# zju3dv/pvnet

Hardware: NVIDIA H100
Metric: images/sec (480x640, K=9) backbone+vote (higher is better)
Workload: dtype tf32 (fp32 storage, fp32 accumulate; vote fp32/fp64)

## Files before the change

### pvnet_b200/csrc/vote.cu

```cuda
#include "common.cuh"

#include <cfloat>
#include <cmath>

namespace {

using pvnet::Carver;

constexpr int CH_PX = 2048;
constexpr int CH_THREADS = 256;
constexpr int VT_THREADS = 256;
constexpr int VT_WARPS = VT_THREADS / 32;
constexpr int VT_TILE = 512;
constexpr int VT_MAX_B = 1024;
constexpr int RF_CHUNKS = 8;
constexpr int RF_THREADS = 256;

struct Strides {
    long long s[5];
};

__device__ __forceinline__ bool exact_inlier(float nx, float ny, float cx, float cy, float hx, float hy,
                                             float thresh)
{
    const float dx = __fsub_rn(hx, cx);
    const float dy = __fsub_rn(hy, cy);
    const float norm1 = __fsqrt_rn(__fmaf_rn(nx, nx, __fmul_rn(ny, ny)));
    const float norm2 = __fsqrt_rn(__fmaf_rn(dx, dx, __fmul_rn(dy, dy)));
    if (fmin((double)norm1, (double)norm2) < 1e-6) return false;
    const float num = __fmaf_rn(dx, nx, __fmul_rn(dy, ny));
    const float den = __fmul_rn(norm1, norm2);
    const float ang = __fdiv_rn(num, den);
    return ang > thresh;
}

__device__ __forceinline__ float2 exact_hypothesis(float d0x, float d0y, float cx0, float cy0, float d1x,
                                                   float d1y, float cx1, float cy1)
{
    const float p = __fmul_rn(d0y, d1x);
    const float q = __fmul_rn(d0x, d1y);
    const float det_y = __fsub_rn(p, q);
    if ((double)fabsf(det_y) < 1e-6) return make_float2(0.f, 0.f);
    const float det_x = __fsub_rn(q, p);
    if ((double)fabsf(det_x) < 1e-6) return make_float2(0.f, 0.f);
    const float s1 = __fmaf_rn(d1y, cx1, -__fmul_rn(d1x, cy1));
    const float s0 = __fmaf_rn(d0y, cx0, -__fmul_rn(d0x, cy0));
    const float y = __fdiv_rn(__fmaf_rn(d1y, s0, -__fmul_rn(d0y, s1)), det_y);
    const float x = __fdiv_rn(__fmaf_rn(-d1x, s0, __fmul_rn(d0x, s1)), det_x);
    return make_float2(x, y);
}

__device__ __forceinline__ int warp_sum(int v)
{
#pragma unroll
    for (int o = 16; o > 0; o >>= 1) v += __shfl_xor_sync(0xffffffffu, v, o);
    return v;
}

__device__ __forceinline__ void block_sum3(int &a, int &b, int &c, int *scratch )
{
    const int lane = threadIdx.x & 31, warp = threadIdx.x >> 5, nw = (blockDim.x + 31) >> 5;
    a = warp_sum(a);
    b = warp_sum(b);
    c = warp_sum(c);
    __syncthreads();
    if (lane == 0) {
        scratch[warp] = a;
        scratch[32 + warp] = b;
        scratch[64 + warp] = c;
    }
    __syncthreads();
    int ta = 0, tb = 0, tc = 0;
    for (int i = 0; i < nw; ++i) {
        ta += scratch[i];
        tb += scratch[32 + i];
        tc += scratch[64 + i];
    }
    a = ta;
    b = tb;
    c = tc;
}

template <typename T>
__device__ __forceinline__ bool is_foreground(T v, int mode)
{
    if (mode == PVNET_MASK_EQUALS_ONE) return v == (T)1;
    return (unsigned char)v != 0;
}

__device__ __forceinline__ float subsample_p(int fg, int max_num)
{
    return __fmul_rn(__frcp_rn((float)fg), (float)max_num);
}

__device__ __forceinline__ uint4 philox4x32_10(uint4 c, uint2 k)
{
#pragma unroll
    for (int r = 0; r < 10; ++r) {
        const unsigned hi0 = __umulhi(0xD2511F53u, c.x), lo0 = 0xD2511F53u * c.x;
        const unsigned hi1 = __umulhi(0xCD9E8D57u, c.z), lo1 = 0xCD9E8D57u * c.z;
        c = make_uint4(hi1 ^ c.y ^ k.x, lo1, hi0 ^ c.w ^ k.y, lo0);
        k.x += 0x9E3779B9u;
        k.y += 0xBB67AE85u;
    }
    return c;
}
enum { RNG_SELECTION = 0, RNG_IDXS_V3 = 1, RNG_IDXS_COV = 2, RNG_IDXS_CENTER = 3 };
__device__ __forceinline__ uint4 rng_draw(const unsigned long long *__restrict__ rng_state, unsigned item,
                                          unsigned image, unsigned stream)
{
    const unsigned long long seed = rng_state[0], off = rng_state[1];
    return philox4x32_10(make_uint4(item, image | (stream << 28), (unsigned)off, (unsigned)(off >> 32)),
                         make_uint2((unsigned)seed, (unsigned)(seed >> 32)));
}
__device__ __forceinline__ float selection_value(const float *__restrict__ sel_field,
                                                 const unsigned long long *__restrict__ rng_state, int b, int npx, int i)
{
    if (sel_field) return sel_field[(size_t)b * npx + i];
    return (float)(rng_draw(rng_state, (unsigned)i, (unsigned)b, RNG_SELECTION).x & 0xffffffu) * 5.9604644775390625e-8f;
}
__global__ void k_rng_bump(unsigned long long *rng_state) { rng_state[1] += 1ull; }

template <typename T>
__global__ void __launch_bounds__(CH_THREADS) k_chunk_count(const T *__restrict__ mask, int mode, int npx,
                                                             int nchunk, int *__restrict__ chunk_fg)
{
    __shared__ int scratch[96];
    const int c = blockIdx.x, b = blockIdx.y;
    const T *m = mask + (size_t)b * npx;
    const int base = c * CH_PX + threadIdx.x * 8;
    int cnt = 0;
#pragma unroll
    for (int j = 0; j < 8; ++j) {
        const int i = base + j;
        if (i < npx) cnt += is_foreground(m[i], mode) ? 1 : 0;
    }
    int z0 = 0, z1 = 0;
    block_sum3(cnt, z0, z1, scratch);
    if (threadIdx.x == 0) chunk_fg[b * nchunk + c] = cnt;
}

template <typename T>
__global__ void __launch_bounds__(CH_THREADS)
    k_chunk_kept(const T *__restrict__ mask, int mode, const float *__restrict__ selection,
                 const unsigned long long *__restrict__ rng_state, int npx, int nchunk, int min_num, int max_num,
                 const int *__restrict__ chunk_fg, int *__restrict__ chunk_kept, int *__restrict__ status)
{
    __shared__ int scratch[96];
    const int c = blockIdx.x, b = blockIdx.y;
    int tot = 0, z0 = 0, z1 = 0;
    for (int i = threadIdx.x; i < nchunk; i += blockDim.x) tot += chunk_fg[b * nchunk + i];
    block_sum3(tot, z0, z1, scratch);
    const bool skip = tot < min_num;
    const bool have_sel = selection != nullptr || rng_state != nullptr;
    const bool sub = tot > max_num && !skip;
    if (!sub || !have_sel) {
        if (threadIdx.x == 0) {
            chunk_kept[b * nchunk + c] = skip ? 0 : chunk_fg[b * nchunk + c];
            if (c == 0) status[b] = (skip ? 1 : 0) | ((sub && !have_sel) ? 4 : 0);
        }
        return;
    }
    const float p = subsample_p(tot, max_num);
    const T *m = mask + (size_t)b * npx;
    const int base = c * CH_PX + threadIdx.x * 8;
    int cnt = 0;
#pragma unroll
    for (int j = 0; j < 8; ++j) {
        const int i = base + j;
        if (i < npx) cnt += (is_foreground(m[i], mode) && selection_value(selection, rng_state, b, npx, i) < p) ? 1 : 0;
    }
    block_sum3(cnt, z0, z1, scratch);
    if (threadIdx.x == 0) {
        chunk_kept[b * nchunk + c] = cnt;
        if (c == 0) status[b] = 2;
    }
}

template <typename T>
__global__ void __launch_bounds__(CH_THREADS)
    k_compact_write(const T *__restrict__ mask, int mode, const float *__restrict__ selection,
                    const unsigned long long *__restrict__ rng_state, int npx, int width, int nchunk, int min_num,
                    int max_num, const int *__restrict__ chunk_fg, const int *__restrict__ chunk_kept_or_null,
                    unsigned *__restrict__ pix, int *__restrict__ tn_out, int *__restrict__ fg_out)
{
    __shared__ int scratch[96];
    __shared__ int warp_off[CH_THREADS / 32];
    const int c = blockIdx.x, b = blockIdx.y;
    const int *chunk_kept = chunk_kept_or_null ? chunk_kept_or_null : chunk_fg;
    int tot_fg = 0, prefix = 0, tot_kept = 0;
    for (int i = threadIdx.x; i < nchunk; i += blockDim.x) {
        const int k = chunk_kept[b * nchunk + i];
        tot_fg += chunk_fg[b * nchunk + i];
        tot_kept += k;
        if (i < c) prefix += k;
    }
    block_sum3(tot_fg, prefix, tot_kept, scratch);
    if (!chunk_kept_or_null && tot_fg < min_num) tot_kept = 0;
    if (c == 0 && threadIdx.x == 0) {
        tn_out[b] = tot_kept;
        fg_out[b] = tot_fg;
    }
    if (tot_kept == 0 || chunk_kept[b * nchunk + c] == 0) return;
    const bool sub = (tot_fg > max_num) && chunk_kept_or_null && (selection != nullptr || rng_state != nullptr);
    const float p = sub ? subsample_p(tot_fg, max_num) : 0.f;
    const T *m = mask + (size_t)b * npx;
    const int base = c * CH_PX + threadIdx.x * 8;
    unsigned flags = 0;
#pragma unroll
    for (int j = 0; j < 8; ++j) {
        const int i = base + j;
        if (i < npx) {
            bool keep = is_foreground(m[i], mode);
            if (sub && keep) keep = selection_value(selection, rng_state, b, npx, i) < p;
            flags |= (keep ? 1u : 0u) << j;
        }
    }
    const int mine = __popc(flags);
    const int lane = threadIdx.x & 31, warp = threadIdx.x >> 5;
    int inc = mine;
#pragma unroll
    for (int o = 1; o < 32; o <<= 1) {
        const int v = __shfl_up_sync(0xffffffffu, inc, o);
        if (lane >= o) inc += v;
    }
    if (lane == 31) warp_off[warp] = inc;
    __syncthreads();
    int woff = 0;
    for (int i = 0; i < warp; ++i) woff += warp_off[i];
    int r = prefix + woff + inc - mine;
    unsigned *out = pix + (size_t)b * npx;
#pragma unroll
    for (int j = 0; j < 8; ++j) {
        if (flags & (1u << j)) {
            const int i = base + j;
            const int y = i / width, x = i - y * width;
            out[r++] = ((unsigned)y << 16) | (unsigned)x;
        }
    }
}

__global__ void k_sum_chunks(const int *__restrict__ chunk_fg, int nchunk, int *__restrict__ fg_out)
{
    __shared__ int scratch[96];
    const int b = blockIdx.x;
    int tot = 0, z0 = 0, z1 = 0;
    for (int i = threadIdx.x; i < nchunk; i += blockDim.x) tot += chunk_fg[b * nchunk + i];
    block_sum3(tot, z0, z1, scratch);
    if (threadIdx.x == 0) fg_out[b] = tot;
}

__global__ void __launch_bounds__(256)
    k_gather(const float *__restrict__ vertex, Strides st, const unsigned *__restrict__ pix,
             const int *__restrict__ tn_arr, int npx, int cap, int vn, float2 *__restrict__ direct)
{
    const int g = blockIdx.x, b = blockIdx.y, tid = threadIdx.x;
    const int tn = tn_arr[b];
    const int t0 = g * VT_TILE;
    if (t0 >= tn) return;
    const int len = min(VT_TILE, tn - t0);
    const bool vec2 = st.s[4] == 1 && ((st.s[0] | st.s[1] | st.s[2] | st.s[3]) & 1) == 0 &&
                      (reinterpret_cast<uintptr_t>(vertex) & 7) == 0;
    for (int i = tid; i < len; i += 256) {
        const unsigned p = pix[(size_t)b * npx + t0 + i];
        const int x = p & 0xffff, y = p >> 16;
        const long long base = (long long)b * st.s[0] + (long long)y * st.s[1] + (long long)x * st.s[2];
        float2 *o = direct + (size_t)b * vn * cap + t0 + i;
        for (int k = 0; k < vn; ++k) {
            const long long off = base + (long long)k * st.s[3];
            float2 v;
            if (vec2) v = __ldg(reinterpret_cast<const float2 *>(vertex + off));
            else v = make_float2(__ldg(vertex + off), __ldg(vertex + off + st.s[4]));
            o[(size_t)k * cap] = v;
        }
    }
}

template <bool SEG>
__device__ __forceinline__ int seg_image(int b, int seg_div) { return SEG ? b / seg_div : b; }
template <bool SEG>
__device__ __forceinline__ int seg_start(const int *seg_off, int b) { return SEG ? seg_off[b] : 0; }

template <bool SEG>
__global__ void __launch_bounds__(256)
    k_gen_hyp(const float2 *__restrict__ direct, const int *__restrict__ idxs,
              const unsigned long long *__restrict__ rng_state, int rng_stream, const unsigned *__restrict__ pix,
              const int *__restrict__ tn_arr, int npx, int cap, int vn, int hn, int HT, int h_off,
              float2 *__restrict__ hyp, const int *__restrict__ seg_off, int seg_div)
{
    const int i = blockIdx.x * blockDim.x + threadIdx.x;
    const int b = blockIdx.y;
    if (i >= hn * vn) return;
    const int hi = i / vn, vi = i - hi * vn;
    const int tn = tn_arr[b];
    float2 out = make_float2(0.f, 0.f);
    if (tn > 0) {
        unsigned t0, t1;
        if (idxs) {
            const size_t ib = (((size_t)b * hn + hi) * vn + vi) * 2;
            t0 = (unsigned)idxs[ib] % (unsigned)tn;
            t1 = (unsigned)idxs[ib + 1] % (unsigned)tn;
        } else {
            const uint4 r = rng_draw(rng_state, (unsigned)i, (unsigned)b, (unsigned)rng_stream);
            t0 = r.x % (unsigned)tn;
            t1 = r.y % (unsigned)tn;
        }
        const int fb = seg_image<SEG>(b, seg_div);
        const int so = seg_start<SEG>(seg_off, b);
        const unsigned *pb = pix + (size_t)fb * npx + so;
        const float2 *db = direct + ((size_t)fb * vn + vi) * cap + so;
        const unsigned p0 = pb[t0], p1 = pb[t1];
        const float2 d0 = db[t0], d1 = db[t1];
        out = exact_hypothesis(d0.x, d0.y, (float)(p0 & 0xffff), (float)(p0 >> 16), d1.x, d1.y, (float)(p1 & 0xffff),
                               (float)(p1 >> 16));
    }
    hyp[((size_t)b * vn + vi) * HT + h_off + hi] = out;
}

typedef unsigned long long f32x2;
__device__ __forceinline__ f32x2 pk2(float a, float b)
{
    f32x2 r;
    asm("mov.b64 %0, {%1, %2};" : "=l"(r) : "f"(a), "f"(b));
    return r;
}
__device__ __forceinline__ void upk2(f32x2 v, float &a, float &b)
{
    asm("mov.b64 {%0, %1}, %2;" : "=f"(a), "=f"(b) : "l"(v));
}
__device__ __forceinline__ f32x2 fma2(f32x2 a, f32x2 b, f32x2 c)
{
    float a0, a1, b0, b1, c0, c1;
    upk2(a, a0, a1);
    upk2(b, b0, b1);
    upk2(c, c0, c1);
    return pk2(__fmaf_rn(a0, b0, c0), __fmaf_rn(a1, b1, c1));
}
__device__ __forceinline__ void lds_2x64(uint32_t addr, f32x2 &a, f32x2 &b)
{
    asm volatile("ld.shared.v2.b64 {%0, %1}, [%2];" : "=l"(a), "=l"(b) : "r"(addr));
}
__device__ __forceinline__ uint32_t ptx_smem_u32(const void *p) { return (uint32_t)__cvta_generic_to_shared(p); }
constexpr int VT_SUB = 64;

__device__ __forceinline__ float min3_nan_abs(float a, float b, float c)
{
    float r;
    asm("{\n\t.reg .f32 t;\n\tmin.NaN.f32 t, %1, %2;\n\tmin.NaN.f32 %0, t, %3;\n\t}" : "=f"(r) : "f"(a), "f"(fabsf(b)), "f"(fabsf(c)));
    return r;
}

template <int HPL, bool SEGMENTED>
__global__ void __launch_bounds__(VT_THREADS, HPL > 4 ? 2 : 3)
    k_vote3(const unsigned *__restrict__ pix, const float2 *__restrict__ direct, const int *__restrict__ tn_arr, int npx,
            int cap, int nb, int vn, int hn, int HT, int h0, const float2 *__restrict__ hyp, int *__restrict__ counts,
            unsigned *__restrict__ ticket, float thresh, float sn, float cs, float beta, float b0, int items_per_warp,
            const int *__restrict__ seg_off, int seg_div)
{
    constexpr int G = 4;
    static_assert(G % 2 == 0 && VT_SUB % G == 0, "pixels are swept in pairs");
    __shared__ float4 rec_all[VT_WARPS * 3 * VT_SUB];
    __shared__ int seg_prefix[VT_MAX_B + 1];
    __shared__ int s_seg;

    const int tid = threadIdx.x, lane = tid & 31, warp = tid >> 5;
    const int HC = 32 * HPL;
    const int hcn = (hn + HC - 1) / HC;
    if (tid == 0) {
        long long px = 0;
        for (int i = 0; i < nb; ++i) px += tn_arr[i];
        const long long want = (long long)gridDim.x * VT_WARPS * items_per_warp;
        int seg = 4096;
        while (seg > 4 * VT_SUB && (px / seg + nb) * vn * hcn < want) seg >>= 1;
        int acc = 0;
        for (int i = 0; i < nb; ++i) {
            seg_prefix[i] = acc;
            acc += (tn_arr[i] + seg - 1) / seg;
        }
        seg_prefix[nb] = acc;
        s_seg = seg;
    }
    __syncthreads();
    const int SEG = s_seg;
    const long long n_items = (long long)seg_prefix[nb] * vn * hcn;
    const float qnan = __int_as_float(0x7fc00000);
    const float finf = __int_as_float(0x7f800000);
    float4 *rec = rec_all + warp * (3 * VT_SUB);
    const uint32_t rec_u = ptx_smem_u32(rec);

    for (;;) {
        unsigned item_u = 0;
        if (lane == 0) item_u = atomicAdd(ticket, 1u);
        const long long it = (long long)__shfl_sync(0xffffffffu, item_u, 0);
        if (it >= n_items) break;
        const int hc = (int)(it % hcn);
        const long long r = it / hcn;
        const int k = (int)(r % vn);
        const int g = (int)(r / vn);
        int lo = 0, hi = nb;
        while (hi - lo > 1) {
            const int mid = (lo + hi) >> 1;
            if (seg_prefix[mid] <= g) lo = mid; else hi = mid;
        }
        const int b = lo;
        const int tn = tn_arr[b];
        const int t0 = (g - seg_prefix[b]) * SEG;
        const int len = min(SEG, tn - t0);
        const int fb = seg_image<SEGMENTED>(b, seg_div);
        const int so = seg_start<SEGMENTED>(seg_off, b) + t0;
        const unsigned *pix_t = pix + (size_t)fb * npx + so;
        const float2 *dir_t = direct + ((size_t)fb * vn + k) * cap + so;

        const int hbase = hc * HC;
        const float2 *hyp_row = hyp + ((size_t)b * vn + k) * HT + h0;
        int *cnt_row = counts + ((size_t)b * vn + k) * HT + h0;
        float2 hraw[HPL];
#pragma unroll
        for (int j = 0; j < HPL; ++j) {
            const int h = hbase + j * 32 + lane;
            hraw[j] = (h < hn) ? __ldg(hyp_row + h) : make_float2(0.f, 0.f);
        }
        unsigned pp[2];
        float2 pn[2];
#pragma unroll
        for (int e = 0; e < 2; ++e) {
            const int i = e * 32 + lane;
            pp[e] = (i < len) ? __ldg(pix_t + i) : 0u;
            pn[e] = (i < len) ? __ldg(dir_t + i) : make_float2(0.f, 0.f);
        }
        int xmin = 0x7fffffff, xmax = -1;
        for (int i = lane; i < len; i += 32) {
            const int x = (int)(__ldg(pix_t + i) & 0xffffu);
            xmin = min(xmin, x);
            xmax = max(xmax, x);
        }
        xmin = __reduce_min_sync(0xffffffffu, xmin);
        xmax = __reduce_max_sync(0xffffffffu, xmax);
        const int ymin = (int)(__ldg(pix_t) >> 16), ymax = (int)(__ldg(pix_t + len - 1) >> 16);
        const float xc = (float)((xmin + xmax) >> 1), yc = (float)((ymin + ymax) >> 1);
        const float r1 = (float)(max((int)xc - xmin, xmax - (int)xc) + max((int)yc - ymin, ymax - (int)yc));

        auto centre = [&](float2 hp, float &hxv, float &hyv, float &bd) {
            hxv = hp.x - xc;
            hyv = hp.y - yc;
            bd = fmaf(beta, fabsf(hxv) + fabsf(hyv) + r1, b0);
            if (!(bd < 1e18f)) bd = qnan;
        };
        f32x2 hx2[HPL / 2], hy2[HPL / 2];
        float bdv[HPL], mab[HPL];
        int cnt[HPL];
#pragma unroll
        for (int j = 0; j < HPL; j += 2) {
            float hxv[2], hyv[2];
#pragma unroll
            for (int e = 0; e < 2; ++e) {
                const int h = hbase + (j + e) * 32 + lane;
                float bd = -1.f;
                hxv[e] = hyv[e] = 0.f;
                if (h < hn) centre(hraw[j + e], hxv[e], hyv[e], bd);
                bdv[j + e] = bd;
                cnt[j + e] = 0;
                mab[j + e] = finf;
            }
            hx2[j / 2] = pk2(hxv[0], hxv[1]);
            hy2[j / 2] = pk2(hyv[0], hyv[1]);
        }

        for (int c0 = 0; c0 < len; c0 += VT_SUB) {
            const int clen = min(VT_SUB, len - c0);
#pragma unroll
            for (int e = 0; e < 2; ++e) {
                const int i = e * 32 + lane;
                const unsigned p = pp[e];
                const float2 n = pn[e];
                const float xr = (float)(int)(p & 0xffff) - xc, yr = (float)(int)(p >> 16) - yc;
                const float n2 = fmaf(n.x, n.x, n.y * n.y);
                const float rinv = rsqrtf(n2);
                const float ux = n.x * rinv, uy = n.y * rinv;
                float sx = sn * ux, sy = sn * uy, cx = -cs * uy, cy = cs * ux;
                float ns = -fmaf(sx, xr, sy * yr), nc = -fmaf(cx, xr, cy * yr);
                if (!(n2 > 1e-11f && n2 < 1e30f)) sx = sy = cx = cy = ns = nc = qnan;
                if (i >= clen) {
                    sx = sy = cx = cy = nc = 0.f;
                    ns = -1e30f;
                }
                rec[3 * i] = make_float4(sx, sx, sy, sy);
                rec[3 * i + 1] = make_float4(ns, ns, cx, cx);
                rec[3 * i + 2] = make_float4(cy, cy, nc, nc);
            }
            __syncwarp();
#pragma unroll
            for (int e = 0; e < 2; ++e) {
                const int i = c0 + VT_SUB + e * 32 + lane;
                pp[e] = (i < len) ? __ldg(pix_t + i) : 0u;
                pn[e] = (i < len) ? __ldg(dir_t + i) : make_float2(0.f, 0.f);
            }
            const int cend = (clen + G - 1) / G * G;
            for (int i0 = 0; i0 < cend; i0 += G) {
                const uint32_t base = rec_u + (uint32_t)i0 * 48u;
#pragma unroll
                for (int u = 0; u < G; u += 2) {
                    f32x2 SX0, SY0, NS0, CX0, CY0, NC0, SX1, SY1, NS1, CX1, CY1, NC1;
                    lds_2x64(base + (uint32_t)u * 48u, SX0, SY0);
                    lds_2x64(base + (uint32_t)u * 48u + 16u, NS0, CX0);
                    lds_2x64(base + (uint32_t)u * 48u + 32u, CY0, NC0);
                    lds_2x64(base + (uint32_t)u * 48u + 48u, SX1, SY1);
                    lds_2x64(base + (uint32_t)u * 48u + 64u, NS1, CX1);
                    lds_2x64(base + (uint32_t)u * 48u + 80u, CY1, NC1);
#pragma unroll
                    for (int j = 0; j < HPL / 2; ++j) {
                        const f32x2 p0 = fma2(hx2[j], SX0, fma2(hy2[j], SY0, NS0));
                        const f32x2 q0 = fma2(hx2[j], CX0, fma2(hy2[j], CY0, NC0));
                        const f32x2 p1 = fma2(hx2[j], SX1, fma2(hy2[j], SY1, NS1));
                        const f32x2 q1 = fma2(hx2[j], CX1, fma2(hy2[j], CY1, NC1));
                        float p0a, p0b, q0a, q0b, p1a, p1b, q1a, q1b;
                        upk2(p0, p0a, p0b);
                        upk2(q0, q0a, q0b);
                        upk2(p1, p1a, p1b);
                        upk2(q1, q1a, q1b);
                        const float e0a = fabsf(q0a) - p0a, e0b = fabsf(q0b) - p0b;
                        const float e1a = fabsf(q1a) - p1a, e1b = fabsf(q1b) - p1b;
                        cnt[2 * j] += (int)(__float_as_uint(e0a) >> 31);
                        cnt[2 * j + 1] += (int)(__float_as_uint(e0b) >> 31);
                        cnt[2 * j] += (int)(__float_as_uint(e1a) >> 31);
                        cnt[2 * j + 1] += (int)(__float_as_uint(e1b) >> 31);
                        mab[2 * j] = min3_nan_abs(mab[2 * j], e0a, e1a);
                        mab[2 * j + 1] = min3_nan_abs(mab[2 * j + 1], e0b, e1b);
                    }
                }
            }
            unsigned fl = 0;
#pragma unroll
            for (int j = 0; j < HPL; ++j) {
                if (!(mab[j] > bdv[j])) fl |= 1u << j;
                mab[j] = finf;
            }
            unsigned lanes = __ballot_sync(0xffffffffu, fl != 0);
            while (lanes) {
                const int src = __ffs(lanes) - 1;
                lanes &= lanes - 1;
                unsigned fm = __shfl_sync(0xffffffffu, fl, src);
                while (fm) {
                    const int j = __ffs(fm) - 1;
                    fm &= fm - 1;
                    const int h = hbase + j * 32 + src;
                    if (h >= hn) continue;
                    const float2 hp = __ldg(hyp_row + h);
                    float hxs, hys, bd;
                    centre(hp, hxs, hys, bd);
                    int add = 0;
#pragma unroll
                    for (int e = 0; e < 2; ++e) {
                        const int pi = e * 32 + lane;
                        if (pi < clen) {
                            const float4 ra = rec[3 * pi], rb = rec[3 * pi + 1], rc = rec[3 * pi + 2];
                            const float num = fmaf(hxs, ra.x, fmaf(hys, ra.z, rb.x));
                            const float perp = fmaf(hxs, rb.z, fmaf(hys, rc.x, rc.z));
                            const float ev = fabsf(perp) - num;
                            if (!(fabsf(ev) > bd)) {
                                const unsigned p = __ldg(pix_t + c0 + pi);
                                const float2 nraw = __ldg(dir_t + c0 + pi);
                                add += (exact_inlier(nraw.x, nraw.y, (float)(p & 0xffff), (float)(p >> 16), hp.x, hp.y, thresh)
                                            ? 1
                                            : 0) -
                                       (int)(__float_as_uint(ev) >> 31);
                            }
                        }
                    }
                    add = __reduce_add_sync(0xffffffffu, add);
                    if (lane == 0 && add) atomicAdd(cnt_row + h, add);
                }
            }
            __syncwarp();
        }

#pragma unroll
        for (int j = 0; j < HPL; ++j) {
            const int h = hbase + j * 32 + lane;
            if (h < hn && cnt[j]) atomicAdd(cnt_row + h, cnt[j]);
        }
    }
}

__device__ __forceinline__ double warp_sum_d(double v)
{
#pragma unroll
    for (int o = 16; o > 0; o >>= 1) v += __shfl_down_sync(0xffffffffu, v, o);
    return v;
}

template <bool SEG>
__global__ void __launch_bounds__(RF_THREADS)
    k_refit(const float2 *__restrict__ direct, int cap, const unsigned *__restrict__ pix,
            const int *__restrict__ tn_arr, int npx, int vn, int hn, int HT, const float2 *__restrict__ hyp,
            const int *__restrict__ counts, float thresh, double *__restrict__ part, float2 *__restrict__ win,
            const float2 *__restrict__ win_in, const int *__restrict__ seg_off, int seg_div)
{
    __shared__ unsigned long long s_key[RF_THREADS / 32];
    __shared__ double s_acc[RF_THREADS / 32][5];
    const int rc = blockIdx.x, bk = blockIdx.y, b = bk / vn, k = bk - b * vn;
    const int tid = threadIdx.x, lane = tid & 31, warp = tid >> 5;
    const int tn = tn_arr[b];
    double *my_part = part + ((size_t)bk * RF_CHUNKS + rc) * 5;
    if (tn == 0) {
        if (tid < 5) my_part[tid] = 0.0;
        if (rc == 0 && tid == 0) win[bk] = make_float2(0.f, 0.f);
        return;
    }
    unsigned long long key = 0;
    for (int h = tid; h < (win_in ? 0 : hn); h += RF_THREADS) {
        const unsigned long long kk =
            ((unsigned long long)(unsigned)counts[(size_t)bk * HT + h] << 32) | (unsigned long long)(0xffffffffu - (unsigned)h);
        key = kk > key ? kk : key;
    }
#pragma unroll
    for (int o = 16; o > 0; o >>= 1) {
        const unsigned long long other = __shfl_xor_sync(0xffffffffu, key, o);
        key = other > key ? other : key;
    }
    if (lane == 0) s_key[warp] = key;
    __syncthreads();
    key = s_key[0];
    for (int i = 1; i < RF_THREADS / 32; ++i) key = s_key[i] > key ? s_key[i] : key;
    const unsigned best_cnt = (unsigned)(key >> 32);
    const unsigned best_h = 0xffffffffu - (unsigned)(key & 0xffffffffu);
    float2 wp = make_float2(0.f, 0.f);
    if (win_in) wp = win_in[bk];
    else if (best_cnt > 0) wp = hyp[(size_t)bk * HT + best_h];
    if (rc == 0 && tid == 0) win[bk] = wp;

    const int per = (tn + RF_CHUNKS - 1) / RF_CHUNKS;
    const int lo = rc * per, hi = min(tn, lo + per);
    const float2 *dir_k = direct + (size_t)bk * cap;
    size_t pix_b = (size_t)b * npx;
    if (SEG) {
        const int so = seg_start<SEG>(seg_off, b), fb = seg_image<SEG>(b, seg_div);
        dir_k = direct + ((size_t)fb * vn + k) * cap + so;
        pix_b = (size_t)fb * npx + so;
    }
    double a00 = 0, a01 = 0, a11 = 0, b0 = 0, b1 = 0;
    for (int t = lo + tid; t < hi; t += RF_THREADS) {
        const unsigned p = pix[pix_b + t];
        const int x = p & 0xffff, y = p >> 16;
        const float2 dv = dir_k[t];
        const float dxv = dv.x, dyv = dv.y;
        if (exact_inlier(dxv, dyv, (float)x, (float)y, wp.x, wp.y, thresh)) {
            const double n0 = (double)dyv, n1 = -(double)dxv;
            const double bb = n0 * (double)x + n1 * (double)y;
            a00 += n0 * n0;
            a01 += n0 * n1;
            a11 += n1 * n1;
            b0 += n0 * bb;
            b1 += n1 * bb;
        }
    }
    a00 = warp_sum_d(a00);
    a01 = warp_sum_d(a01);
    a11 = warp_sum_d(a11);
    b0 = warp_sum_d(b0);
    b1 = warp_sum_d(b1);
    if (lane == 0) {
        s_acc[warp][0] = a00;
        s_acc[warp][1] = a01;
        s_acc[warp][2] = a11;
        s_acc[warp][3] = b0;
        s_acc[warp][4] = b1;
    }
    __syncthreads();
    if (tid < 5) {
        double v = 0;
        for (int i = 0; i < RF_THREADS / 32; ++i) v += s_acc[i][tid];
        my_part[tid] = v;
    }
}

__global__ void k_refit_final(const double *__restrict__ part, const int *__restrict__ tn_arr, int nb, int vn,
                              float *__restrict__ out_pts)
{
    const int bk = blockIdx.x * blockDim.x + threadIdx.x;
    if (bk >= nb * vn) return;
    const int b = bk / vn;
    float px = 0.f, py = 0.f;
    if (tn_arr[b] > 0) {
        double a[5] = {0, 0, 0, 0, 0};
        for (int rc = 0; rc < RF_CHUNKS; ++rc)
            for (int i = 0; i < 5; ++i) a[i] += part[((size_t)bk * RF_CHUNKS + rc) * 5 + i];
        const double det = a[0] * a[2] - a[1] * a[1];
        px = (float)((a[2] * a[3] - a[1] * a[4]) / det);
        py = (float)((a[0] * a[4] - a[1] * a[3]) / det);
    }
    out_pts[bk * 2] = px;
    out_pts[bk * 2 + 1] = py;
}

__global__ void __launch_bounds__(RF_THREADS)
    k_conf_count(const float2 *__restrict__ direct, int cap, const unsigned *__restrict__ pix,
                 const int *__restrict__ tn_arr, int npx, int vn, const float *__restrict__ pts, float thresh,
                 int *__restrict__ conf_cnt)
{
    __shared__ int scratch[96];
    const int rc = blockIdx.x, bk = blockIdx.y, b = bk / vn;
    const int tn = tn_arr[b];
    if (tn == 0) return;
    const float hx = pts[bk * 2], hy = pts[bk * 2 + 1];
    const int per = (tn + RF_CHUNKS - 1) / RF_CHUNKS;
    const int lo = rc * per, hi = min(tn, lo + per);
    const float2 *dir_k = direct + (size_t)bk * cap;
    int c = 0, z0 = 0, z1 = 0;
    for (int t = lo + threadIdx.x; t < hi; t += RF_THREADS) {
        const unsigned p = pix[(size_t)b * npx + t];
        const int x = p & 0xffff, y = p >> 16;
        const float2 dv = dir_k[t];
        c += exact_inlier(dv.x, dv.y, (float)x, (float)y, hx, hy, thresh) ? 1 : 0;
    }
    block_sum3(c, z0, z1, scratch);
    if (threadIdx.x == 0 && c) atomicAdd(conf_cnt + bk, c);
}

__global__ void k_conf_final(const int *__restrict__ conf_cnt, const int *__restrict__ tn_arr, int nb, int vn,
                             float *__restrict__ out_conf)
{
    const int bk = blockIdx.x * blockDim.x + threadIdx.x;
    if (bk >= nb * vn) return;
    const int tn = tn_arr[bk / vn];
    out_conf[bk] = tn > 0 ? __fdiv_rn((float)conf_cnt[bk], (float)tn) : 0.f;
}

__device__ __forceinline__ void block_sum2_d(double &a, double &b, double (*s_acc)[2])
{
    const int lane = threadIdx.x & 31, warp = threadIdx.x >> 5;
    a = warp_sum_d(a);
    b = warp_sum_d(b);
    if (lane == 0) {
        s_acc[warp][0] = a;
        s_acc[warp][1] = b;
    }
    __syncthreads();
    if (threadIdx.x == 0) {
        a = b = 0.0;
        for (int i = 0; i < RF_THREADS / 32; ++i) {
            a += s_acc[i][0];
            b += s_acc[i][1];
        }
    }
}

__global__ void __launch_bounds__(RF_THREADS)
    k_resid_sum(const float2 *__restrict__ direct, int cap, const unsigned *__restrict__ pix,
                const int *__restrict__ tn_arr, int npx, int vn, const float2 *__restrict__ win,
                const float *__restrict__ pts, float thresh, double *__restrict__ part)
{
    __shared__ double s_acc[RF_THREADS / 32][2];
    const int rc = blockIdx.x, bk = blockIdx.y, b = bk / vn;
    const int tn = tn_arr[b];
    double *my_part = part + ((size_t)bk * RF_CHUNKS + rc) * 2;
    double r2 = 0.0, cnt = 0.0;
    if (tn > 0) {
        const float2 wp = win[bk];
        const double px = (double)pts[bk * 2], py = (double)pts[bk * 2 + 1];
        const int per = (tn + RF_CHUNKS - 1) / RF_CHUNKS;
        const int lo = rc * per, hi = min(tn, lo + per);
        const float2 *dir_k = direct + (size_t)bk * cap;
        for (int t = lo + threadIdx.x; t < hi; t += RF_THREADS) {
            const unsigned p = pix[(size_t)b * npx + t];
            const int x = p & 0xffff, y = p >> 16;
            const float2 dv = dir_k[t];
            const float dxv = dv.x, dyv = dv.y;
            if (exact_inlier(dxv, dyv, (float)x, (float)y, wp.x, wp.y, thresh)) {
                const double n0 = (double)dyv, n1 = -(double)dxv;
                const double r = n0 * px + n1 * py - (n0 * (double)x + n1 * (double)y);
                r2 += r * r;
                cnt += 1.0;
            }
        }
    }
    block_sum2_d(r2, cnt, s_acc);
    if (threadIdx.x == 0) {
        my_part[0] = r2;
        my_part[1] = cnt;
    }
}

__global__ void k_resid_final(const double *__restrict__ part, const int *__restrict__ tn_arr, int nb, int vn,
                              float *__restrict__ out_var)
{
    const int bk = blockIdx.x * blockDim.x + threadIdx.x;
    if (bk >= nb * vn) return;
    float v = 1.f;
    if (tn_arr[bk / vn] > 0) {
        double r2 = 0.0, cnt = 0.0;
        for (int rc = 0; rc < RF_CHUNKS; ++rc) {
            r2 += part[((size_t)bk * RF_CHUNKS + rc) * 2];
            cnt += part[((size_t)bk * RF_CHUNKS + rc) * 2 + 1];
        }
        v = (float)(r2 / cnt);
    }
    out_var[bk] = v;
}

__global__ void __launch_bounds__(RF_THREADS)
    k_motion_sum(const float2 *__restrict__ direct, int cap, const unsigned *__restrict__ pix,
                 const int *__restrict__ tn_arr, int npx, int vn, double *__restrict__ part)
{
    __shared__ double s_acc[RF_THREADS / 32][2];
    const int rc = blockIdx.x, bk = blockIdx.y, b = bk / vn;
    const int tn = tn_arr[b];
    double sx = 0.0, sy = 0.0;
    const int per = (tn + RF_CHUNKS - 1) / RF_CHUNKS;
    const int lo = rc * per, hi = min(tn, lo + per);
    const float2 *dir_k = direct + (size_t)bk * cap;
    for (int t = lo + threadIdx.x; t < hi; t += RF_THREADS) {
        const unsigned p = pix[(size_t)b * npx + t];
        const int x = p & 0xffff, y = p >> 16;
        const float2 dv = dir_k[t];
        sx += (double)__fadd_rn(dv.x, (float)x);
        sy += (double)__fadd_rn(dv.y, (float)y);
    }
    block_sum2_d(sx, sy, s_acc);
    if (threadIdx.x == 0) {
        double *my_part = part + ((size_t)bk * RF_CHUNKS + rc) * 2;
        my_part[0] = sx;
        my_part[1] = sy;
    }
}

__global__ void k_motion_final(const double *__restrict__ part, const int *__restrict__ tn_arr, int nb, int vn,
                               float *__restrict__ out_pts)
{
    const int bk = blockIdx.x * blockDim.x + threadIdx.x;
    if (bk >= nb * vn) return;
    const int tn = tn_arr[bk / vn];
    float px = 0.f, py = 0.f;
    if (tn > 0) {
        double sx = 0.0, sy = 0.0;
        for (int rc = 0; rc < RF_CHUNKS; ++rc) {
            sx += part[((size_t)bk * RF_CHUNKS + rc) * 2];
            sy += part[((size_t)bk * RF_CHUNKS + rc) * 2 + 1];
        }
        px = (float)(sx / (double)tn);
        py = (float)(sy / (double)tn);
    }
    out_pts[bk * 2] = px;
    out_pts[bk * 2 + 1] = py;
}

__global__ void k_export(const float2 *__restrict__ hyp, const int *__restrict__ counts,
                         const int *__restrict__ tn_arr, int nb, int vn, int hn, int HT, int h_off,
                         float *__restrict__ out_hyp, int *__restrict__ out_counts, int *__restrict__ out_tn)
{
    const long long n = (long long)nb * vn * hn;
    for (long long i = (long long)blockIdx.x * blockDim.x + threadIdx.x; i < n;
         i += (long long)gridDim.x * blockDim.x) {
        const int k = (int)(i % vn);
        const long long r = i / vn;
        const int h = (int)(r % hn);
        const int b = (int)(r / hn);
        const size_t src = ((size_t)b * vn + k) * HT + h_off + h;
        if (out_counts) out_counts[i] = counts[src];
        if (out_hyp) {
            const float2 v = hyp[src];
            out_hyp[i * 2] = v.x;
            out_hyp[i * 2 + 1] = v.y;
        }
    }
// ... 1246 lines not shown
```

Before: 1718.

## Compact vote record layout, cache hypotheses in smem, vectorize mask loads

The vote kernel drops the emulated packed-pair FMA path, whose shared-memory records stored every value twice. Records are now stored once as float2 and read as float4, halving per-warp record space, and the pixel sweep group grows from 4 to 8. Hypotheses and per-lane pixel/direction values are kept in shared memory and registers for the exact-recheck path instead of being reloaded from global memory. The mask counting and compaction kernels read 8 byte-sized mask values with one 64-bit load when alignment allows. The extra hypothesis buffer adds shared memory and register pressure, which could lower occupancy.

```diff
diff --git a/pvnet_b200/csrc/vote.cu b/pvnet_b200/csrc/vote.cu
--- a/pvnet_b200/csrc/vote.cu
+++ b/pvnet_b200/csrc/vote.cu
@@ -88,6 +88,29 @@
     return (unsigned char)v != 0;
 }
 
+template <typename T>
+__device__ __forceinline__ unsigned foreground_flags8(const T *__restrict__ m, int base, int npx, int mode)
+{
+    unsigned f = 0;
+    if constexpr (sizeof(T) == 1) {
+        if (base + 8 <= npx && (reinterpret_cast<uintptr_t>(m + base) & 7) == 0) {
+            const uint2 v = __ldg(reinterpret_cast<const uint2 *>(m + base));
+#pragma unroll
+            for (int j = 0; j < 8; ++j) {
+                const T byte = (T)(((j < 4 ? v.x : v.y) >> (8 * (j & 3))) & 0xffu);
+                f |= (is_foreground(byte, mode) ? 1u : 0u) << j;
+            }
+            return f;
+        }
+    }
+#pragma unroll
+    for (int j = 0; j < 8; ++j) {
+        const int i = base + j;
+        if (i < npx) f |= (is_foreground(m[i], mode) ? 1u : 0u) << j;
+    }
+    return f;
+}
+
 __device__ __forceinline__ float subsample_p(int fg, int max_num)
 {
     return __fmul_rn(__frcp_rn((float)fg), (float)max_num);
@@ -129,12 +152,7 @@
     const int c = blockIdx.x, b = blockIdx.y;
     const T *m = mask + (size_t)b * npx;
     const int base = c * CH_PX + threadIdx.x * 8;
-    int cnt = 0;
-#pragma unroll
-    for (int j = 0; j < 8; ++j) {
-        const int i = base + j;
-        if (i < npx) cnt += is_foreground(m[i], mode) ? 1 : 0;
-    }
+    int cnt = __popc(foreground_flags8(m, base, npx, mode));
     int z0 = 0, z1 = 0;
     block_sum3(cnt, z0, z1, scratch);
     if (threadIdx.x == 0) chunk_fg[b * nchunk + c] = cnt;
@@ -206,15 +224,11 @@
     const float p = sub ? subsample_p(tot_fg, max_num) : 0.f;
     const T *m = mask + (size_t)b * npx;
     const int base = c * CH_PX + threadIdx.x * 8;
-    unsigned flags = 0;
-#pragma unroll
-    for (int j = 0; j < 8; ++j) {
-        const int i = base + j;
-        if (i < npx) {
-            bool keep = is_foreground(m[i], mode);
-            if (sub && keep) keep = selection_value(selection, rng_state, b, npx, i) < p;
-            flags |= (keep ? 1u : 0u) << j;
-        }
+    unsigned flags = foreground_flags8(m, base, npx, mode);
+    if (sub) {
+#pragma unroll
+        for (int j = 0; j < 8; ++j)
+            if ((flags >> j & 1u) && !(selection_value(selection, rng_state, b, npx, base + j) < p)) flags &= ~(1u << j);
     }
     const int mine = __popc(flags);
     const int lane = threadIdx.x & 31, warp = threadIdx.x >> 5;
@@ -317,30 +331,6 @@
     hyp[((size_t)b * vn + vi) * HT + h_off + hi] = out;
 }
 
-typedef unsigned long long f32x2;
-__device__ __forceinline__ f32x2 pk2(float a, float b)
-{
-    f32x2 r;
-    asm("mov.b64 %0, {%1, %2};" : "=l"(r) : "f"(a), "f"(b));
-    return r;
-}
-__device__ __forceinline__ void upk2(f32x2 v, float &a, float &b)
-{
-    asm("mov.b64 {%0, %1}, %2;" : "=f"(a), "=f"(b) : "l"(v));
-}
-__device__ __forceinline__ f32x2 fma2(f32x2 a, f32x2 b, f32x2 c)
-{
-    float a0, a1, b0, b1, c0, c1;
-    upk2(a, a0, a1);
-    upk2(b, b0, b1);
-    upk2(c, c0, c1);
-    return pk2(__fmaf_rn(a0, b0, c0), __fmaf_rn(a1, b1, c1));
-}
-__device__ __forceinline__ void lds_2x64(uint32_t addr, f32x2 &a, f32x2 &b)
-{
-    asm volatile("ld.shared.v2.b64 {%0, %1}, [%2];" : "=l"(a), "=l"(b) : "r"(addr));
-}
-__device__ __forceinline__ uint32_t ptx_smem_u32(const void *p) { return (uint32_t)__cvta_generic_to_shared(p); }
 constexpr int VT_SUB = 64;
 
 __device__ __forceinline__ float min3_nan_abs(float a, float b, float c)
@@ -357,9 +347,10 @@
             unsigned *__restrict__ ticket, float thresh, float sn, float cs, float beta, float b0, int items_per_warp,
             const int *__restrict__ seg_off, int seg_div)
 {
-    constexpr int G = 4;
+    constexpr int G = 8;
     static_assert(G % 2 == 0 && VT_SUB % G == 0, "pixels are swept in pairs");
-    __shared__ float4 rec_all[VT_WARPS * 3 * VT_SUB];
+    __shared__ float4 rec_all[VT_WARPS * 3 * VT_SUB / 2];
+    __shared__ float2 hyp_all[VT_WARPS * 32 * HPL];
     __shared__ int seg_prefix[VT_MAX_B + 1];
     __shared__ int s_seg;
 
@@ -385,8 +376,9 @@
     const long long n_items = (long long)seg_prefix[nb] * vn * hcn;
     const float qnan = __int_as_float(0x7fc00000);
     const float finf = __int_as_float(0x7f800000);
-    float4 *rec = rec_all + warp * (3 * VT_SUB);
-    const uint32_t rec_u = ptx_smem_u32(rec);
+    const float4 *rec4 = rec_all + warp * (3 * VT_SUB / 2);
+    float2 *rec = reinterpret_cast<float2 *>(rec_all + warp * (3 * VT_SUB / 2));
+    float2 *hyp_w = hyp_all + warp * (32 * HPL);
 
     for (;;) {
         unsigned item_u = 0;
@@ -419,6 +411,7 @@
         for (int j = 0; j < HPL; ++j) {
             const int h = hbase + j * 32 + lane;
             hraw[j] = (h < hn) ? __ldg(hyp_row + h) : make_float2(0.f, 0.f);
+            hyp_w[j * 32 + lane] = hraw[j];
         }
         unsigned pp[2];
         float2 pn[2];
@@ -446,33 +439,31 @@
             bd = fmaf(beta, fabsf(hxv) + fabsf(hyv) + r1, b0);
             if (!(bd < 1e18f)) bd = qnan;
         };
-        f32x2 hx2[HPL / 2], hy2[HPL / 2];
+        float hx[HPL], hy[HPL];
         float bdv[HPL], mab[HPL];
         int cnt[HPL];
 #pragma unroll
-        for (int j = 0; j < HPL; j += 2) {
-            float hxv[2], hyv[2];
-#pragma unroll
-            for (int e = 0; e < 2; ++e) {
-                const int h = hbase + (j + e) * 32 + lane;
-                float bd = -1.f;
-                hxv[e] = hyv[e] = 0.f;
-                if (h < hn) centre(hraw[j + e], hxv[e], hyv[e], bd);
-                bdv[j + e] = bd;
-                cnt[j + e] = 0;
-                mab[j + e] = finf;
-            }
-            hx2[j / 2] = pk2(hxv[0], hxv[1]);
-            hy2[j / 2] = pk2(hyv[0], hyv[1]);
+        for (int j = 0; j < HPL; ++j) {
+            const int h = hbase + j * 32 + lane;
+            float bd = -1.f;
+            hx[j] = hy[j] = 0.f;
+            if (h < hn) centre(hraw[j], hx[j], hy[j], bd);
+            bdv[j] = bd;
+            cnt[j] = 0;
+            mab[j] = finf;
         }
 
         for (int c0 = 0; c0 < len; c0 += VT_SUB) {
             const int clen = min(VT_SUB, len - c0);
+            unsigned pcur[2];
+            float2 ncur[2];
 #pragma unroll
             for (int e = 0; e < 2; ++e) {
                 const int i = e * 32 + lane;
                 const unsigned p = pp[e];
                 const float2 n = pn[e];
+                pcur[e] = p;
+                ncur[e] = n;
                 const float xr = (float)(int)(p & 0xffff) - xc, yr = (float)(int)(p >> 16) - yc;
                 const float n2 = fmaf(n.x, n.x, n.y * n.y);
                 const float rinv = rsqrtf(n2);
@@ -484,9 +475,9 @@
                     sx = sy = cx = cy = nc = 0.f;
                     ns = -1e30f;
                 }
-                rec[3 * i] = make_float4(sx, sx, sy, sy);
-                rec[3 * i + 1] = make_float4(ns, ns, cx, cx);
-                rec[3 * i + 2] = make_float4(cy, cy, nc, nc);
+                rec[3 * i] = make_float2(sx, sy);
+                rec[3 * i + 1] = make_float2(ns, cx);
+                rec[3 * i + 2] = make_float2(cy, nc);
             }
             __syncwarp();
 #pragma unroll
@@ -497,35 +488,20 @@
             }
             const int cend = (clen + G - 1) / G * G;
             for (int i0 = 0; i0 < cend; i0 += G) {
-                const uint32_t base = rec_u + (uint32_t)i0 * 48u;
-#pragma unroll
-                for (int u = 0; u < G; u += 2) {
-                    f32x2 SX0, SY0, NS0, CX0, CY0, NC0, SX1, SY1, NS1, CX1, CY1, NC1;
-                    lds_2x64(base + (uint32_t)u * 48u, SX0, SY0);
-                    lds_2x64(base + (uint32_t)u * 48u + 16u, NS0, CX0);
-                    lds_2x64(base + (uint32_t)u * 48u + 32u, CY0, NC0);
-                    lds_2x64(base + (uint32_t)u * 48u + 48u, SX1, SY1);
-                    lds_2x64(base + (uint32_t)u * 48u + 64u, NS1, CX1);
-                    lds_2x64(base + (uint32_t)u * 48u + 80u, CY1, NC1);
-#pragma unroll
-                    for (int j = 0; j < HPL / 2; ++j) {
-                        const f32x2 p0 = fma2(hx2[j], SX0, fma2(hy2[j], SY0, NS0));
-                        const f32x2 q0 = fma2(hx2[j], CX0, fma2(hy2[j], CY0, NC0));
-                        const f32x2 p1 = fma2(hx2[j], SX1, fma2(hy2[j], SY1, NS1));
-                        const f32x2 q1 = fma2(hx2[j], CX1, fma2(hy2[j], CY1, NC1));
-                        float p0a, p0b, q0a, q0b, p1a, p1b, q1a, q1b;
-                        upk2(p0, p0a, p0b);
-                        upk2(q0, q0a, q0b);
-                        upk2(p1, p1a, p1b);
-                        upk2(q1, q1a, q1b);
-                        const float e0a = fabsf(q0a) - p0a, e0b = fabsf(q0b) - p0b;
-                        const float e1a = fabsf(q1a) - p1a, e1b = fabsf(q1b) - p1b;
-                        cnt[2 * j] += (int)(__float_as_uint(e0a) >> 31);
-                        cnt[2 * j + 1] += (int)(__float_as_uint(e0b) >> 31);
-                        cnt[2 * j] += (int)(__float_as_uint(e1a) >> 31);
-                        cnt[2 * j + 1] += (int)(__float_as_uint(e1b) >> 31);
-                        mab[2 * j] = min3_nan_abs(mab[2 * j], e0a, e1a);
-                        mab[2 * j + 1] = min3_nan_abs(mab[2 * j + 1], e0b, e1b);
+                const float4 *rp = rec4 + (i0 >> 1) * 3;
+#pragma unroll
+                for (int u = 0; u < G / 2; ++u) {
+                    const float4 a = rp[3 * u], bq = rp[3 * u + 1], cq = rp[3 * u + 2];
+#pragma unroll
+                    for (int j = 0; j < HPL; ++j) {
+                        const float p0 = fmaf(hx[j], a.x, fmaf(hy[j], a.y, a.z));
+                        const float q0 = fmaf(hx[j], a.w, fmaf(hy[j], bq.x, bq.y));
+                        const float p1 = fmaf(hx[j], bq.z, fmaf(hy[j], bq.w, cq.x));
+                        const float q1 = fmaf(hx[j], cq.y, fmaf(hy[j], cq.z, cq.w));
+                        const float e0 = fabsf(q0) - p0, e1 = fabsf(q1) - p1;
+                        cnt[j] += (int)(__float_as_uint(e0) >> 31);
+                        cnt[j] += (int)(__float_as_uint(e1) >> 31);
+                        mab[j] = min3_nan_abs(mab[j], e0, e1);
                     }
                 }
             }
@@ -545,7 +521,7 @@
                     fm &= fm - 1;
                     const int h = hbase + j * 32 + src;
                     if (h >= hn) continue;
-                    const float2 hp = __ldg(hyp_row + h);
+                    const float2 hp = hyp_w[j * 32 + src];
                     float hxs, hys, bd;
                     centre(hp, hxs, hys, bd);
                     int add = 0;
@@ -553,13 +529,13 @@
                     for (int e = 0; e < 2; ++e) {
                         const int pi = e * 32 + lane;
                         if (pi < clen) {
-                            const float4 ra = rec[3 * pi], rb = rec[3 * pi + 1], rc = rec[3 * pi + 2];
-                            const float num = fmaf(hxs, ra.x, fmaf(hys, ra.z, rb.x));
-                            const float perp = fmaf(hxs, rb.z, fmaf(hys, rc.x, rc.z));
+                            const float2 ra = rec[3 * pi], rb = rec[3 * pi + 1], rc = rec[3 * pi + 2];
+                            const float num = fmaf(hxs, ra.x, fmaf(hys, ra.y, rb.x));
+                            const float perp = fmaf(hxs, rb.y, fmaf(hys, rc.x, rc.y));
                             const float ev = fabsf(perp) - num;
                             if (!(fabsf(ev) > bd)) {
-                                const unsigned p = __ldg(pix_t + c0 + pi);
-                                const float2 nraw = __ldg(dir_t + c0 + pi);
+                                const unsigned p = pcur[e];
+                                const float2 nraw = ncur[e];
                                 add += (exact_inlier(nraw.x, nraw.y, (float)(p & 0xffff), (float)(p >> 16), hp.x, hp.y, thresh)
                                             ? 1
                                             : 0) -
```

Result: no change. 1720 (median of 6 runs) (+0.1%).
